# OxfordML/GPz

Measured on AMD Instinct MI355X. Metric: objective+gradient evals/sec, higher is better.
Workload: dtype f64

## Files before the change

### gpz_amd/csrc/k_phi_quad.hip

```cpp
#include <float.h>
#include "gpz_dev.h"
#include "gpz_kernels.h"

template <int D>
struct PhiQuadShape {
    static constexpr int NT = D * (D + 1) / 2;
    static constexpr int NF = 1 + D + NT;
    static constexpr int NK = (NF + 3) / 4;
    static constexpr int CS = 4 * NK;
};

int phi_quad_stride(int de) { return 4 * ((1 + de + de * (de + 1) / 2 + 3) / 4); }
bool phi_quad_fits(int kind, int de, int mp, int k) { return kind == GPZ_KIND_COV && (de == 8 || de == 10) && mp > 256 && k == 1; }

template <int D>
__global__ __launch_bounds__(64) void k_phi_quad_coef(const double *__restrict__ Rc, const double *__restrict__ P,
                                                        const double *__restrict__ xmu, const double *__restrict__ fmx, int m, int mp,
                                                        double *__restrict__ Cq, double *__restrict__ blockmax,
                                                        unsigned *__restrict__ ticket, double *__restrict__ bound,
                                                        int *__restrict__ route) {
    constexpr int NT = PhiQuadShape<D>::NT, NF = PhiQuadShape<D>::NF, CS = PhiQuadShape<D>::CS, NP = NT + D;
    const int j = blockIdx.x * 64 + threadIdx.x;
    double bj = 0.0;
    if (j < m) {
        double R[NT], pq[D], u[D], uh[D];
        const double *rj = Rc + (size_t)j * NP;
#pragma unroll
        for (int e = 0; e < NT; ++e) R[e] = rj[e];
#pragma unroll
        for (int a = 0; a < D; ++a) pq[a] = P[(size_t)j * D + a] - xmu[a];
#pragma unroll
        for (int a = 0; a < D; ++a) {
            double s = 0.0, sh = 0.0;
#pragma unroll
            for (int b = a; b < D; ++b) {
                const double r = R[a * D - a * (a - 1) / 2 + (b - a)];
                s = fma(r, pq[b], s);
                sh = fma(fabs(r), fabs(pq[b]), sh);
            }
            u[a] = s; uh[a] = sh;
        }
        double *o = Cq + (size_t)j * CS;
        double c0 = 0.0, c0h = 0.0;
#pragma unroll
        for (int a = 0; a < D; ++a) { c0 = fma(u[a], u[a], c0); c0h = fma(uh[a], uh[a], c0h); }
        o[0] = -0.5 * c0;
        double bs = fmx[0] * (0.5 * c0h);
#pragma unroll
        for (int a = 0; a < D; ++a) {
            double s = 0.0, sh = 0.0;
#pragma unroll
            for (int r = 0; r <= a; ++r) {
                const double v = R[r * D - r * (r - 1) / 2 + (a - r)];
                s = fma(v, u[r], s);
                sh = fma(fabs(v), uh[r], sh);
            }
            o[1 + a] = s;
            bs = fma(fmx[1 + a], sh, bs);
        }
#pragma unroll
        for (int a = 0; a < D; ++a)
#pragma unroll
            for (int b = a; b < D; ++b) {
                double s = 0.0, sh = 0.0;
#pragma unroll
                for (int r = 0; r <= a; ++r) {
                    const double va = R[r * D - r * (r - 1) / 2 + (a - r)], vb = R[r * D - r * (r - 1) / 2 + (b - r)];
                    s = fma(va, vb, s);
                    sh = fma(fabs(va), fabs(vb), sh);
                }
                const int f = 1 + D + a * D - a * (a - 1) / 2 + (b - a);
                const double sc = (a == b) ? 0.5 : 1.0;
                o[f] = -sc * s;
                bs = fma(fmx[f], sc * sh, bs);
            }
#pragma unroll
        for (int f = NF; f < CS; ++f) o[f] = 0.0;
        bj = (double)(NF + 2 * D + 6) * 0x1p-53 * bs;
        if (!(bj <= DBL_MAX)) bj = __longlong_as_double(0x7ff0000000000000LL);
    } else if (j < mp) {
        double *o = Cq + (size_t)j * CS;
#pragma unroll
        for (int f = 0; f < CS; ++f) o[f] = 0.0;
    }
#pragma unroll
    for (int off = 32; off > 0; off >>= 1) bj = fmax(bj, __shfl_xor(bj, off, 64));
    int last = 0;
    if (threadIdx.x == 0) {
        blockmax[blockIdx.x] = bj;
        __threadfence();
        last = atomicAdd(ticket, 1u) == gridDim.x - 1 ? 1 : 0;
        if (last) {
            __threadfence();
            double mx = 0.0;
            for (unsigned g = 0; g < gridDim.x; ++g) mx = fmax(mx, __hip_atomic_load(blockmax + g, __ATOMIC_RELAXED, __HIP_MEMORY_SCOPE_AGENT));
            *bound = mx;
            *route = mx <= GPZ_PHI_QUAD_TAU ? GPZ_PHI_ROUTE_QUAD : GPZ_PHI_ROUTE_EXACT;
            *ticket = 0u;
        }
    }
}

int launch_phi_quad_coef(hipStream_t st, const double *Rc, const double *P, const double *xmu, const double *fmx, int m, int mp, int de,
                         double *Cq, double *blockmax, unsigned *ticket, double *bound, int *route) {
    dim3 g((mp + 63) / 64), b(64);
    switch (de) {
        case 8: hipLaunchKernelGGL(k_phi_quad_coef<8>, g, b, 0, st, Rc, P, xmu, fmx, m, mp, Cq, blockmax, ticket, bound, route); break;
        case 10: hipLaunchKernelGGL(k_phi_quad_coef<10>, g, b, 0, st, Rc, P, xmu, fmx, m, mp, Cq, blockmax, ticket, bound, route); break;
        default: return -1;
    }
    return 0;
}

struct PhiQuadKArgs {
    const double *Xs;
    const double *Cq;
    const int *route;
    int n, m, mp;
    const double *v, *bvec, *omega, *Y;
    double *Phi, *lnbeta, *wbeta;
    int jgroup;
    double *part;
    long ldp;
};

#ifndef GPZ_PHI_QUAD_RB
#define GPZ_PHI_QUAD_RB 2
#endif
#ifndef GPZ_PHI_QUAD_WGS
#define GPZ_PHI_QUAD_WGS 3
#endif

template <int D, int RB>
__global__ __launch_bounds__(256, GPZ_PHI_QUAD_WGS) void k_phi_quad(PhiQuadKArgs a) {
    constexpr int NF = PhiQuadShape<D>::NF, NK = PhiQuadShape<D>::NK, CS = PhiQuadShape<D>::CS, XL = D + 2;
    constexpr int NPB = 16 * CS;
    constexpr int NLD = (NPB + 255) / 256;
    if (*a.route != GPZ_PHI_ROUTE_QUAD) return;
    __shared__ double cq[2][NPB];
    __shared__ unsigned char pia[CS], pib[CS];
    const int tid = threadIdx.x, lane = tid & 63, wave = tid >> 6, li = lane & 15, lk = lane >> 4;
    const long row0 = ((long)blockIdx.x * 4 + wave) * (16 * RB);

    if (tid < CS) {
        const int f = tid;
        int ia = 0, ib = 0;
        if (f >= NF) ia = ib = XL - 1;
        else if (f >= 1) {
            if (f <= D) ia = f;
            else {
                int e2 = f - 1 - D, aa = 0;
                while (e2 >= D - aa) { e2 -= D - aa; ++aa; }
                ia = aa + 1; ib = aa + e2 + 1;
            }
        }
        pia[f] = (unsigned char)ia; pib[f] = (unsigned char)ib;
    }
    const int jlo = blockIdx.y * a.jgroup;
    const int jhi = min(a.mp, jlo + a.jgroup);
    double stg[NLD];
    auto pload = [&](int j0) {
#pragma unroll
        for (int q = 0; q < NLD; ++q) {
            const int e = tid + 256 * q;
            stg[q] = e < NPB ? a.Cq[(size_t)j0 * CS + e] : 0.0;
        }
    };
    auto pstore = [&](int buf) {
#pragma unroll
        for (int q = 0; q < NLD; ++q) {
            const int e = tid + 256 * q;
            if (e < NPB) cq[buf][e] = stg[q];
        }
    };
    pload(jlo);
    pstore(0);
    __syncthreads();

    double F[RB][NK];
#pragma unroll
    for (int ks = 0; ks < NK; ++ks) {
        const int ia = pia[4 * ks + lk], ib = pib[4 * ks + lk];
#pragma unroll
        for (int rb = 0; rb < RB; ++rb) {
            const long i = row0 + 16 * rb + li;
            const double *xr = a.Xs + (size_t)i * XL;
            F[rb][ks] = xr[ia] * xr[ib];
        }
    }
    double sv[RB][4];
#pragma unroll
    for (int rb = 0; rb < RB; ++rb)
#pragma unroll
        for (int r = 0; r < 4; ++r) sv[rb][r] = 0.0;

    int cur = 0;
    for (int j0 = jlo; j0 < jhi; j0 += 16, cur ^= 1) {
        const bool more = j0 + 16 < jhi;
        if (more) pload(j0 + 16);
        const int j = j0 + li;
        const double vj = (a.v && j < a.m) ? a.v[j] : 0.0;
        d4_t acc[RB];
#pragma unroll
        for (int rb = 0; rb < RB; ++rb) acc[rb] = d4_t{0.0, 0.0, 0.0, 0.0};
        const double *cb = &cq[cur][li * CS + lk];
#pragma unroll
        for (int ks = 0; ks < NK; ++ks) {
            const double b = cb[4 * ks];
#pragma unroll
            for (int rb = 0; rb < RB; ++rb) acc[rb] = MFMA_F64(F[rb][ks], b, acc[rb]);
        }
        double ph[RB][4];
#pragma unroll
        for (int rb = 0; rb < RB; ++rb) {
#pragma unroll
            for (int r = 0; r < 4; ++r) {
                const long i = row0 + 16 * rb + lk + 4 * r;
                const double e = exp(fmin(acc[rb][r], 0.0));
                ph[rb][r] = i < a.n ? e : 0.0;
                sv[rb][r] = fma(ph[rb][r], vj, sv[rb][r]);
            }
        }
        if (j0 + 16 > a.m) {
#pragma unroll
            for (int rb = 0; rb < RB; ++rb) {
#pragma unroll
                for (int r = 0; r < 4; ++r) {
                    const double y = a.Y ? a.Y[row0 + 16 * rb + lk + 4 * r] : 0.0;
                    if (j >= a.m) ph[rb][r] = j == a.m ? y : 0.0;
                }
            }
        }
        double *const po = a.Phi + (size_t)(row0 + lk) * a.mp + j;
#pragma unroll
        for (int rb = 0; rb < RB; ++rb) {
#pragma unroll
            for (int r = 0; r < 4; ++r) po[(size_t)(16 * rb + 4 * r) * a.mp] = ph[rb][r];
        }
        if (more) pstore(cur ^ 1);
        __syncthreads();
    }

#pragma unroll
    for (int rb = 0; rb < RB; ++rb)
#pragma unroll
        for (int r = 0; r < 4; ++r) {
#pragma unroll
            for (int off = 1; off < 16; off <<= 1) sv[rb][r] += __shfl_xor(sv[rb][r], off, 64);
        }
    if (li != 0) return;
#pragma unroll
    for (int rb = 0; rb < RB; ++rb)
#pragma unroll
        for (int r = 0; r < 4; ++r) {
            const long i = row0 + 16 * rb + lk + 4 * r;
            if (a.part) {
                if (i < a.ldp) {
                    a.part[((size_t)blockIdx.y * 2 + 0) * a.ldp + i] = sv[rb][r];
                    a.part[((size_t)blockIdx.y * 2 + 1) * a.ldp + i] = 0.0;
                }
                continue;
            }
            const bool valid = i < a.n;
            const double lb = a.bvec[0] + sv[rb][r];
            a.lnbeta[i] = valid ? lb : 0.0;
            if (a.wbeta) {
                const double om = a.omega ? a.omega[i] : 1.0;
                a.wbeta[i] = valid ? om * exp(-lb) : 0.0;
            }
        }
}

template <int D>
static int launch_phi_quad_d(hipStream_t st, const PhiArgs &a, const double *Xs, const double *Cq) {
    constexpr int RB = GPZ_PHI_QUAD_RB, JB = 16;
    const int rows_per_wg = 4 * 16 * RB;
    if (a.n_pad <= 0 || a.n_pad % rows_per_wg != 0 || a.n_pad > a.ldx) return -1;
    const int nwg = a.n_pad / rows_per_wg;
    int ngroup = 1;
    if (a.part && nwg < 1024) {
        int maxg = a.mp / (4 * JB);
        if (maxg > a.part_groups) maxg = a.part_groups;
        ngroup = phi_pick_groups(nwg, a.mp, JB, 2, 16, maxg < 1 ? 1 : maxg);
    }
    int jgroup = ((a.mp + ngroup - 1) / ngroup + JB - 1) / JB * JB;
    ngroup = (a.mp + jgroup - 1) / jgroup;
    PhiQuadKArgs q{};
    q.Xs = Xs; q.Cq = Cq; q.route = a.route; q.n = a.n; q.m = a.m; q.mp = a.mp;
    q.v = a.v; q.bvec = a.b; q.omega = a.omega; q.Y = a.Y;
    q.Phi = a.Phi; q.lnbeta = a.lnbeta; q.wbeta = a.wbeta;
    q.jgroup = jgroup; q.part = ngroup > 1 ? a.part : nullptr; q.ldp = (long)a.n_pad;
    hipLaunchKernelGGL((k_phi_quad<D, RB>), dim3(nwg, ngroup), dim3(256), 0, st, q);
    if (q.part)
        launch_phi_finalize(st, q.part, ngroup, a, a.route, GPZ_PHI_ROUTE_QUAD);
    return hipGetLastError() == hipSuccess ? 0 : -1;
}

int launch_phi_quad(hipStream_t st, const PhiArgs &a, const double *Xs, const double *Cq) {
    if (a.k != 1 || a.mp % 16 != 0 || !a.route || a.wgtab || !a.Phi || !a.lnbeta || a.w || a.phiw) return -1;
    switch (a.d) {
        case 8: return launch_phi_quad_d<8>(st, a, Xs, Cq);
        case 10: return launch_phi_quad_d<10>(st, a, Xs, Cq);
        default: return -1;
    }
}
```

Before: 18.99.

## Use custom table-based exp for nonpositive args and specialize row-guard path

Replaces the library exp in the quadratic Phi kernel with a table-driven exp valid for nonpositive inputs, with the 64-entry table staged in LDS. The inner loop is split into guarded and unguarded variants so full blocks skip the per-row bounds check. Global loads and stores switch to precomputed byte offsets held in VGPRs, and the wave index is made scalar via readfirstlane. The custom exp trades library handling of special cases for fewer instructions, and it adds extra LDS traffic and code size.

```diff
diff --git a/gpz_amd/csrc/gpz_exp_nonpos.h b/gpz_amd/csrc/gpz_exp_nonpos.h
--- /dev/null
+++ b/gpz_amd/csrc/gpz_exp_nonpos.h
@@ -0,0 +1,124 @@
+#pragma once
+#include <math.h>
+#include <stdint.h>
+#include <string.h>
+
+#if defined(__HIPCC__)
+#define GPZ_EXP_FN __host__ __device__ __forceinline__
+#else
+#define GPZ_EXP_FN static inline
+#endif
+
+#define GPZ_EXP_INVL  0x1.71547652b82fep+6
+#define GPZ_EXP_LHI   0x1.62e42fefa39efp-7
+#define GPZ_EXP_LLO   0x1.abc9e3b39803fp-62
+#define GPZ_EXP_C2    0x1.fffffffffd5fap-2
+#define GPZ_EXP_C3    0x1.5555555554954p-3
+#define GPZ_EXP_C4    0x1.55557621e124fp-5
+#define GPZ_EXP_C5    0x1.111123cf17a63p-7
+#define GPZ_EXP_MAGIC 0x1.8p+52
+#define GPZ_EXP_XMIN  -1024.0
+#define GPZ_EXP_XMIN_HI 0xC0900000u
+
+#define GPZ_EXP_TAB \
+    {0x1.0000000000000p+0, 0x0.0p+0}, \
+    {0x1.02c9a3e778061p+0, -0x1.19083535b085dp-56}, \
+    {0x1.059b0d3158574p+0, 0x1.d73e2a475b465p-55}, \
+    {0x1.0874518759bc8p+0, 0x1.186be4bb284ffp-57}, \
+    {0x1.0b5586cf9890fp+0, 0x1.8a62e4adc610bp-54}, \
+    {0x1.0e3ec32d3d1a2p+0, 0x1.03a1727c57b53p-59}, \
+    {0x1.11301d0125b51p+0, -0x1.6c51039449b3ap-54}, \
+    {0x1.1429aaea92de0p+0, -0x1.32fbf9af1369ep-54}, \
+    {0x1.172b83c7d517bp+0, -0x1.19041b9d78a76p-55}, \
+    {0x1.1a35beb6fcb75p+0, 0x1.e5b4c7b4968e4p-55}, \
+    {0x1.1d4873168b9aap+0, 0x1.e016e00a2643cp-54}, \
+    {0x1.2063b88628cd6p+0, 0x1.dc775814a8495p-55}, \
+    {0x1.2387a6e756238p+0, 0x1.9b07eb6c70573p-54}, \
+    {0x1.26b4565e27cddp+0, 0x1.2bd339940e9d9p-55}, \
+    {0x1.29e9df51fdee1p+0, 0x1.612e8afad1255p-55}, \
+    {0x1.2d285a6e4030bp+0, 0x1.0024754db41d5p-54}, \
+    {0x1.306fe0a31b715p+0, 0x1.6f46ad23182e4p-55}, \
+    {0x1.33c08b26416ffp+0, 0x1.32721843659a6p-54}, \
+    {0x1.371a7373aa9cbp+0, -0x1.63aeabf42eae2p-54}, \
+    {0x1.3a7db34e59ff7p+0, -0x1.5e436d661f5e3p-56}, \
+    {0x1.3dea64c123422p+0, 0x1.ada0911f09ebcp-55}, \
+    {0x1.4160a21f72e2ap+0, -0x1.ef3691c309278p-58}, \
+    {0x1.44e086061892dp+0, 0x1.89b7a04ef80d0p-59}, \
+    {0x1.486a2b5c13cd0p+0, 0x1.3c1a3b69062f0p-56}, \
+    {0x1.4bfdad5362a27p+0, 0x1.d4397afec42e2p-56}, \
+    {0x1.4f9b2769d2ca7p+0, -0x1.4b309d25957e3p-54}, \
+    {0x1.5342b569d4f82p+0, -0x1.07abe1db13cadp-55}, \
+    {0x1.56f4736b527dap+0, 0x1.9bb2c011d93adp-54}, \
+    {0x1.5ab07dd485429p+0, 0x1.6324c054647adp-54}, \
+    {0x1.5e76f15ad2148p+0, 0x1.ba6f93080e65ep-54}, \
+    {0x1.6247eb03a5585p+0, -0x1.383c17e40b497p-54}, \
+    {0x1.6623882552225p+0, -0x1.bb60987591c34p-54}, \
+    {0x1.6a09e667f3bcdp+0, -0x1.bdd3413b26456p-54}, \
+    {0x1.6dfb23c651a2fp+0, -0x1.bbe3a683c88abp-57}, \
+    {0x1.71f75e8ec5f74p+0, -0x1.16e4786887a99p-55}, \
+    {0x1.75feb564267c9p+0, -0x1.0245957316dd3p-54}, \
+    {0x1.7a11473eb0187p+0, -0x1.41577ee04992fp-55}, \
+    {0x1.7e2f336cf4e62p+0, 0x1.05d02ba15797ep-56}, \
+    {0x1.82589994cce13p+0, -0x1.d4c1dd41532d8p-54}, \
+    {0x1.868d99b4492edp+0, -0x1.fc6f89bd4f6bap-54}, \
+    {0x1.8ace5422aa0dbp+0, 0x1.6e9f156864b27p-54}, \
+    {0x1.8f1ae99157736p+0, 0x1.5cc13a2e3976cp-55}, \
+    {0x1.93737b0cdc5e5p+0, -0x1.75fc781b57ebcp-57}, \
+    {0x1.97d829fde4e50p+0, -0x1.d185b7c1b85d1p-54}, \
+    {0x1.9c49182a3f090p+0, 0x1.c7c46b071f2bep-56}, \
+    {0x1.a0c667b5de565p+0, -0x1.359495d1cd533p-54}, \
+    {0x1.a5503b23e255dp+0, -0x1.d2f6edb8d41e1p-54}, \
+    {0x1.a9e6b5579fdbfp+0, 0x1.0fac90ef7fd31p-54}, \
+    {0x1.ae89f995ad3adp+0, 0x1.7a1cd345dcc81p-54}, \
+    {0x1.b33a2b84f15fbp+0, -0x1.2805e3084d708p-57}, \
+    {0x1.b7f76f2fb5e47p+0, -0x1.5584f7e54ac3bp-56}, \
+    {0x1.bcc1e904bc1d2p+0, 0x1.23dd07a2d9e84p-55}, \
+    {0x1.c199bdd85529cp+0, 0x1.11065895048ddp-55}, \
+    {0x1.c67f12e57d14bp+0, 0x1.2884dff483cadp-54}, \
+    {0x1.cb720dcef9069p+0, 0x1.503cbd1e949dbp-56}, \
+    {0x1.d072d4a07897cp+0, -0x1.cbc3743797a9cp-54}, \
+    {0x1.d5818dcfba487p+0, 0x1.2ed02d75b3707p-55}, \
+    {0x1.da9e603db3285p+0, 0x1.c2300696db532p-54}, \
+    {0x1.dfc97337b9b5fp+0, -0x1.1a5cd4f184b5cp-54}, \
+    {0x1.e502ee78b3ff6p+0, 0x1.39e8980a9cc8fp-55}, \
+    {0x1.ea4afa2a490dap+0, -0x1.e9c23179c2893p-54}, \
+    {0x1.efa1bee615a27p+0, 0x1.dc7f486a4b6b0p-54}, \
+    {0x1.f50765b6e4540p+0, 0x1.9d3e12dd8a18bp-54}, \
+    {0x1.fa7c1819e90d8p+0, 0x1.74853f3a5931ep-55}
+
+struct alignas(16) gpz_exp_pair { double hi, lo; };
+
+__attribute__((unused)) static const gpz_exp_pair gpz_exp_tab_host[64] = {GPZ_EXP_TAB};
+#if defined(__HIPCC__)
+__attribute__((unused)) static __constant__ gpz_exp_pair gpz_exp_tab_dev[64] = {GPZ_EXP_TAB};
+#endif
+
+GPZ_EXP_FN double gpz_exp_nonpos_tab(double x, const gpz_exp_pair *tab) {
+    uint64_t xb;
+    memcpy(&xb, &x, 8);
+    uint32_t xh = (uint32_t)(xb >> 32);
+    xh = x < GPZ_EXP_XMIN ? GPZ_EXP_XMIN_HI : xh;
+    xb = ((uint64_t)xh << 32) | (xb & 0xffffffffu);
+    memcpy(&x, &xb, 8);
+    const double kd = fma(x, GPZ_EXP_INVL, GPZ_EXP_MAGIC);
+    const double k = kd - GPZ_EXP_MAGIC;
+    uint64_t kb;
+    memcpy(&kb, &kd, 8);
+    const int32_t ki = (int32_t)(uint32_t)kb;
+    double r = fma(k, -GPZ_EXP_LHI, x);
+    r = fma(k, -GPZ_EXP_LLO, r);
+    const gpz_exp_pair t = tab[ki & 63];
+    double q = fma(GPZ_EXP_C5, r, GPZ_EXP_C4);
+    q = fma(q, r, GPZ_EXP_C3);
+    q = fma(q, r, GPZ_EXP_C2);
+    const double p = fma(q, r * r, r);
+    return ldexp(t.hi + fma(t.hi, p, t.lo), ki >> 6);
+}
+
+GPZ_EXP_FN double gpz_exp_nonpos(double x) {
+#if defined(__HIP_DEVICE_COMPILE__)
+    return gpz_exp_nonpos_tab(x, gpz_exp_tab_dev);
+#else
+    return gpz_exp_nonpos_tab(x, gpz_exp_tab_host);
+#endif
+}
diff --git a/gpz_amd/csrc/k_phi_quad.hip b/gpz_amd/csrc/k_phi_quad.hip
--- a/gpz_amd/csrc/k_phi_quad.hip
+++ b/gpz_amd/csrc/k_phi_quad.hip
@@ -1,5 +1,7 @@
 #include <float.h>
+#include <type_traits>
 #include "gpz_dev.h"
+#include "gpz_exp_nonpos.h"
 #include "gpz_kernels.h"
 
 template <int D>
@@ -138,9 +140,11 @@
     constexpr int NLD = (NPB + 255) / 256;
     if (*a.route != GPZ_PHI_ROUTE_QUAD) return;
     __shared__ double cq[2][NPB];
+    __shared__ gpz_exp_pair etab[64];
     __shared__ unsigned char pia[CS], pib[CS];
-    const int tid = threadIdx.x, lane = tid & 63, wave = tid >> 6, li = lane & 15, lk = lane >> 4;
+    const int tid = threadIdx.x, lane = tid & 63, wave = __builtin_amdgcn_readfirstlane(tid >> 6), li = lane & 15, lk = lane >> 4;
     const long row0 = ((long)blockIdx.x * 4 + wave) * (16 * RB);
+    if (tid < 64) etab[tid] = gpz_exp_tab_dev[tid];
 
     if (tid < CS) {
         const int f = tid;
@@ -159,11 +163,14 @@
     const int jlo = blockIdx.y * a.jgroup;
     const int jhi = min(a.mp, jlo + a.jgroup);
     double stg[NLD];
+    unsigned vcq = (unsigned)tid * 8;
     auto pload = [&](int j0) {
+        const char *pc = reinterpret_cast<const char *>(a.Cq + (size_t)j0 * CS);
 #pragma unroll
         for (int q = 0; q < NLD; ++q) {
             const int e = tid + 256 * q;
-            stg[q] = e < NPB ? a.Cq[(size_t)j0 * CS + e] : 0.0;
+            asm volatile("" : "+v"(vcq));
+            stg[q] = (256 * (q + 1) <= NPB || e < NPB) ? *reinterpret_cast<const double *>(pc + 2048 * q + vcq) : 0.0;
         }
     };
     auto pstore = [&](int buf) {
@@ -194,52 +201,71 @@
 #pragma unroll
         for (int r = 0; r < 4; ++r) sv[rb][r] = 0.0;
 
-    int cur = 0;
-    for (int j0 = jlo; j0 < jhi; j0 += 16, cur ^= 1) {
-        const bool more = j0 + 16 < jhi;
-        if (more) pload(j0 + 16);
-        const int j = j0 + li;
-        const double vj = (a.v && j < a.m) ? a.v[j] : 0.0;
-        d4_t acc[RB];
-#pragma unroll
-        for (int rb = 0; rb < RB; ++rb) acc[rb] = d4_t{0.0, 0.0, 0.0, 0.0};
-        const double *cb = &cq[cur][li * CS + lk];
-#pragma unroll
-        for (int ks = 0; ks < NK; ++ks) {
-            const double b = cb[4 * ks];
-#pragma unroll
-            for (int rb = 0; rb < RB; ++rb) acc[rb] = MFMA_F64(F[rb][ks], b, acc[rb]);
-        }
-        double ph[RB][4];
-#pragma unroll
-        for (int rb = 0; rb < RB; ++rb) {
-#pragma unroll
-            for (int r = 0; r < 4; ++r) {
-                const long i = row0 + 16 * rb + lk + 4 * r;
-                const double e = exp(fmin(acc[rb][r], 0.0));
-                ph[rb][r] = i < a.n ? e : 0.0;
-                sv[rb][r] = fma(ph[rb][r], vj, sv[rb][r]);
-            }
-        }
-        if (j0 + 16 > a.m) {
+    unsigned vst[4];
+#pragma unroll
+    for (int r = 0; r < 4; ++r) vst[r] = (unsigned)(((4 * r + lk) * a.mp + li) * 8);
+    const size_t bst = (size_t)a.mp * (16 * 8);
+    auto steps = [&](auto guard) {
+        constexpr bool GUARD = decltype(guard)::value;
+        char *pst = reinterpret_cast<char *>(a.Phi + (size_t)row0 * a.mp + jlo);
+        int cur = 0;
+        for (int j0 = jlo; j0 < jhi; j0 += 16, cur ^= 1) {
+            const bool more = j0 + 16 < jhi;
+            if (more) pload(j0 + 16);
+            const int j = j0 + li;
+            const double vj = (a.v && j < a.m) ? a.v[j] : 0.0;
+            d4_t acc[RB];
+#pragma unroll
+            for (int rb = 0; rb < RB; ++rb) acc[rb] = d4_t{0.0, 0.0, 0.0, 0.0};
+            const double *cb = &cq[cur][li * CS + lk];
+#pragma unroll
+            for (int ks = 0; ks < NK; ++ks) {
+                const double b = cb[4 * ks];
+#pragma unroll
+                for (int rb = 0; rb < RB; ++rb) acc[rb] = MFMA_F64(F[rb][ks], b, acc[rb]);
+            }
+            double ph[RB][4];
 #pragma unroll
             for (int rb = 0; rb < RB; ++rb) {
 #pragma unroll
                 for (int r = 0; r < 4; ++r) {
-                    const double y = a.Y ? a.Y[row0 + 16 * rb + lk + 4 * r] : 0.0;
-                    if (j >= a.m) ph[rb][r] = j == a.m ? y : 0.0;
-                }
-            }
-        }
-        double *const po = a.Phi + (size_t)(row0 + lk) * a.mp + j;
-#pragma unroll
-        for (int rb = 0; rb < RB; ++rb) {
-#pragma unroll
-            for (int r = 0; r < 4; ++r) po[(size_t)(16 * rb + 4 * r) * a.mp] = ph[rb][r];
-        }
-        if (more) pstore(cur ^ 1);
-        __syncthreads();
-    }
+                    const double e = gpz_exp_nonpos_tab(fmin(acc[rb][r], 0.0), etab);
+                    if (GUARD) {
+                        const long i = row0 + 16 * rb + lk + 4 * r;
+                        ph[rb][r] = i < a.n ? e : 0.0;
+                    } else
+                        ph[rb][r] = e;
+                    sv[rb][r] = fma(ph[rb][r], vj, sv[rb][r]);
+                }
+                if (D == 8) __builtin_amdgcn_sched_barrier(0);
+            }
+#pragma unroll
+            for (int rb = 0; rb < RB; ++rb) {
+#pragma unroll
+                for (int r = 0; r < 4; ++r) {
+                    asm volatile("" : "+v"(vst[r]));
+                    *reinterpret_cast<double *>(pst + rb * bst + vst[r]) = ph[rb][r];
+                }
+            }
+            if (j0 + 16 > a.m) {
+                if (j >= a.m) {
+#pragma unroll
+                    for (int rb = 0; rb < RB; ++rb) {
+#pragma unroll
+                        for (int r = 0; r < 4; ++r) {
+                            const double y = a.Y ? a.Y[row0 + 16 * rb + lk + 4 * r] : 0.0;
+                            *reinterpret_cast<double *>(pst + rb * bst + vst[r]) = j == a.m ? y : 0.0;
+                        }
+                    }
+                }
+            }
+            pst += 16 * 8;
+            if (more) pstore(cur ^ 1);
+            __syncthreads();
+        }
+    };
+    if (((long)blockIdx.x + 1) * (64 * RB) > (long)a.n) steps(std::true_type{});
+    else steps(std::false_type{});
 
 #pragma unroll
     for (int rb = 0; rb < RB; ++rb)
```

After: 19.03 (median of 6 runs). About the same (+0.2%).
